# cmhungsteve/TA3N

Measured on NVIDIA H100. Metric: video-clips/sec fwd+bwd (B=256,T=5,D=2048), higher is better.
Workload: dtype tf32x3

## Files before the change

### ta3n_b200/csrc/gemm_wgmma.cuh

```cuda
#pragma once

#include <cuda.h>
#include <stdlib.h>

#include <algorithm>
#include <cmath>
#include <functional>
#include <map>
#include <tuple>

#include "seg_gemm.cuh"

namespace ta3n {

constexpr int TC_BM = 128, TC_BN = 128, TC_BK = 32;
constexpr int TC_THREADS = 288;
constexpr int TC_CONSUMER_WARPS = 8;
constexpr int TC_A_BYTES = TC_BM * TC_BK * 4;
constexpr int TC_B_BYTES = TC_BN * TC_BK * 4;
constexpr int TC_STAGE_BYTES = TC_A_BYTES + TC_B_BYTES;
constexpr int TC_STAGES = 4;
constexpr int tc_smem_bytes(int stages) { return stages * TC_STAGE_BYTES + 1024; }
constexpr int TC_ACC_LD = TC_BN + 4;
constexpr int TC_ACC_BYTES = TC_BM * TC_ACC_LD * 4;
static_assert(TC_ACC_BYTES <= TC_STAGES * TC_STAGE_BYTES, "the per-launch kernel reuses its operand ring");
#ifndef TA3N_MAX_MAPS
#define TA3N_MAX_MAPS 64
#endif
constexpr int kMaxMaps = TA3N_MAX_MAPS;

struct alignas(64) TcMaps {
  CUtensorMap m[kMaxMaps];
};
struct TcSegMaps {
  unsigned char a[kMaxSegs];
  unsigned char b[kMaxSegs];
};

__device__ __forceinline__ uint32_t smem_u32(const void* p) { return (uint32_t)__cvta_generic_to_shared(p); }

// ... 9 lines not shown
  do {
    asm volatile(
        "{\n\t.reg .pred p;\n\t"
        "mbarrier.try_wait.parity.shared::cta.b64 p, [%1], %2;\n\t"
        "selp.u32 %0, 1, 0, p;\n\t}"
        : "=r"(done)
        : "r"(addr), "r"(parity)
        : "memory");
  } while (!done);
}
__device__ __forceinline__ void mbar_arrive(uint64_t* bar) {
  asm volatile("mbarrier.arrive.shared::cta.b64 _, [%0];" ::"r"(smem_u32(bar)) : "memory");
}
__device__ __forceinline__ void fence_barrier_init() { asm volatile("fence.mbarrier_init.release.cluster;" ::: "memory"); }
__device__ __forceinline__ void fence_proxy_async() { asm volatile("fence.proxy.async.shared::cta;" ::: "memory"); }
__device__ __forceinline__ void consumer_sync() { asm volatile("bar.sync 1, 256;" ::: "memory"); }

__device__ __forceinline__ void tma_load_2d(void* smem_dst, const CUtensorMap* map, uint64_t* bar, int c0, int c1) {
  asm volatile(
      "cp.async.bulk.tensor.2d.shared::cluster.global.mbarrier::complete_tx::bytes [%0], [%1, {%3, %4}], [%2];"
      ::"r"(smem_u32(smem_dst)), "l"(map), "r"(smem_u32(bar)), "r"(c0), "r"(c1)
      : "memory");
}
__device__ __forceinline__ void tma_load_3d(void* smem_dst, const CUtensorMap* map, uint64_t* bar, int c0, int c1,
                                            int c2) {
  asm volatile(
      "cp.async.bulk.tensor.3d.shared::cluster.global.mbarrier::complete_tx::bytes [%0], [%1, {%3, %4, %5}], [%2];"
      ::"r"(smem_u32(smem_dst)), "l"(map), "r"(smem_u32(bar)), "r"(c0), "r"(c1), "r"(c2)
      : "memory");
}
__device__ __forceinline__ void tma_prefetch_2d(const CUtensorMap* map, int c0, int c1) {
// ... 71 lines not shown
  *kq = ((t >> 1) & 3) | (((t >> 7) & 1) << 2);
}
__device__ __forceinline__ void tc_prep_load(const uint32_t base, const int t, float4 (&r)[4]) {
  int mq, kq;
  tc_prep_blk(t, &mq, &kq);
#pragma unroll
  for (int i = 0; i < 4; ++i) r[i] = lds4(base + mnmaj_chunk(4 * kq + i, mq));
}
__device__ __forceinline__ void tc_prep_store(const uint32_t base, const int t, const float4 (&r)[4]) {
  int mq, kq;
  tc_prep_blk(t, &mq, &kq);
#pragma unroll
  for (int i = 0; i < 4; ++i)
    sts4(base + kmaj_chunk(4 * mq + i, kq), make_float4(f4_at(r[0], i), f4_at(r[1], i), f4_at(r[2], i), f4_at(r[3], i)));
}
__device__ __forceinline__ void tc_prep_stage(const uint32_t a_base, const uint32_t b_base, const bool a_kmaj,
                                              const bool b_kmaj) {
  if (a_kmaj && b_kmaj) return;
  const int t = threadIdx.x;
  float4 ra[4], rb[4];
  if (!a_kmaj) tc_prep_load(a_base, t, ra);
  if (!b_kmaj) tc_prep_load(b_base, t, rb);
  consumer_sync();
  if (!a_kmaj) tc_prep_store(a_base, t, ra);
  if (!b_kmaj) tc_prep_store(b_base, t, rb);
  fence_proxy_async();
  consumer_sync();
}

__device__ __forceinline__ void tc_store_acc(float* acc, const float (&d)[64], const int t) {
  const int lane = t & 31;
  const int row0 = (t >> 7) * 64 + ((t >> 5) & 3) * 16 + (lane >> 2);
#pragma unroll
  for (int j = 0; j < 16; ++j)
#pragma unroll
    for (int h = 0; h < 2; ++h)
      *reinterpret_cast<float2*>(acc + (row0 + 8 * h) * TC_ACC_LD + 8 * j + 2 * (lane & 3)) =
          make_float2(d[4 * j + 2 * h], d[4 * j + 2 * h + 1]);
}
__device__ __forceinline__ void acc_ld_32(const float* acc, int row, int col0, float* v) {
  const float* p = acc + row * TC_ACC_LD + col0;
#pragma unroll
  for (int j = 0; j < 32; j += 4) {
    const float4 q = *reinterpret_cast<const float4*>(p + j);
    v[j] = q.x;
    v[j + 1] = q.y;
    v[j + 2] = q.z;
    v[j + 3] = q.w;
  }
}

struct TcShared {
  uint64_t full_bar[4];
  uint64_t empty_bar[4];
};

template <int STAGES>
__device__ __forceinline__ void tc_pipe_init(TcShared* sh) {
  for (int s = 0; s < STAGES; ++s) {
    mbar_init(&sh->full_bar[s], 1);
    mbar_init(&sh->empty_bar[s], TC_CONSUMER_WARPS);
  }
  fence_barrier_init();
}

enum : int { TILE_FINAL = 0, TILE_PARTIAL = 1 };

template <int STAGES, int STAGE_BYTES = TC_STAGE_BYTES>
__device__ __forceinline__ void tc_produce(const TileCtx& ctx, const CUtensorMap* __restrict__ maps, const bool a_kmaj,
                                           const bool b_kmaj, const int pad_flags, const int m0, const int n0,
                                           const int c_begin, const int n_iter, uint8_t* smem, TcShared* sh,
                                           const uint32_t slabs) {
  const Group& g = ctx.g;
  int seg = 0, k0 = 0;
  {
    int skip = c_begin;
    while (seg < g.seg_count) {
      const int nch = (ctx.seg[seg].len + TC_BK - 1) / TC_BK;
      if (skip < nch) {
        k0 = skip * TC_BK;
        break;
// ... 24 lines not shown
      tma_load_2d(sB, mb, &sh->full_bar[stage], k0, n0);
    } else if (pad_flags & 2) {
      tma_load_3d(sB, mb, &sh->full_bar[stage], 0, k0, n0 >> 5);
    } else {
#pragma unroll
      for (int q = 0; q < TC_BN / 32; ++q) tma_load_2d(sB + q * 4096, mb, &sh->full_bar[stage], n0 + 32 * q, k0);
    }
    k0 += TC_BK;
    if (k0 >= ctx.seg[seg].len) {
      ++seg;
      k0 = 0;
    }
  }
}

template <int STAGES>
__device__ __forceinline__ void tc_consume(const bool a_kmaj, const bool b_kmaj, const int n_iter, uint8_t* smem,
                                           TcShared* sh, float (&d)[64]) {
  const int wg = threadIdx.x >> 7, lane = threadIdx.x & 31;
#pragma unroll
  for (int j = 0; j < 64; ++j) d[j] = 0.f;
  int prev = -1;
  for (int it = 0; it < n_iter; ++it) {
    const uint32_t gl = (uint32_t)it;
    const int stage = (int)(gl % STAGES);
    mbar_wait(&sh->full_bar[stage], (gl / STAGES) & 1u);
    const uint32_t a_base = smem_u32(smem + stage * TC_STAGE_BYTES);
    const uint32_t b_base = a_base + TC_A_BYTES;
    tc_prep_stage(a_base, b_base, a_kmaj, b_kmaj);
    wgmma_fence();
#pragma unroll
    for (int ks = 0; ks < TC_BK / 8; ++ks) wgmma_tf32(d, wgmma_desc(a_base + wg * 64 * 128, ks), wgmma_desc(b_base, ks));
    wgmma_commit();
    wgmma_wait<1>();
    if (prev >= 0) {
      __syncwarp();
      if (lane == 0) mbar_arrive(&sh->empty_bar[prev]);
    }
    prev = stage;
  }
  wgmma_wait<0>();
  if (prev >= 0) {
    __syncwarp();
    if (lane == 0) mbar_arrive(&sh->empty_bar[prev]);
  }
}

template <int kEpiWarps>
__device__ __forceinline__ void tc_epilogue(const TileCtx& ctx, const int m0, const int n0, const int split,
                                            const int n_iter, const int mode, const float* acc, const int ew) {
  const int lane = threadIdx.x & 31;
  const int lq = ew & 3;
  const Group e = ctx.g;
  const int m = m0 + lq * 32 + lane;
  const bool split_out = mode == TILE_PARTIAL;
  float* const obase = split_out ? e.partial + (size_t)split * e.M * e.N : e.C;
  const int ldo = split_out ? e.N : e.ldc;
  constexpr int kColChunks = (TC_BN / 32) * 4 / kEpiWarps;
  const int c0 = (ew / 4) * kColChunks;
#pragma unroll 1
  for (int c = c0; c < c0 + kColChunks; ++c) {
    float v[32];
    if (n_iter > 0) {
      acc_ld_32(acc, lq * 32 + lane, c * 32, v);
    } else {
#pragma unroll
      for (int j = 0; j < 32; ++j) v[j] = 0.f;
    }
    const int nb = n0 + c * 32;
    if (m < e.M && nb < e.N) {
      float* orow = obase + (size_t)m * ldo + nb;
      const int nvalid = min(32, e.N - nb);
      if (!split_out) {
        TA3N_EPI_DISPATCH(e.flags, { epilogue_row32<EPI_F>(e, m, nb, nvalid, v); })
      }
      if (nb + 32 <= e.N && ((reinterpret_cast<uintptr_t>(orow) & 15u) == 0)) {
#pragma unroll
        for (int j = 0; j < 32; j += 4)
          *reinterpret_cast<float4*>(orow + j) = make_float4(v[j], v[j + 1], v[j + 2], v[j + 3]);
      } else {
#pragma unroll
        for (int j = 0; j < 32; ++j)
          if (nb + j < e.N) orow[j] = v[j];
      }
    }
  }
}

__device__ __forceinline__ void tc_chunk_range(const TileCtx& ctx, int split, int* c_begin, int* n_iter) {
  const Group& g = ctx.g;
  int total_chunks = 0;
  for (int s = 0; s < g.seg_count; ++s) total_chunks += (ctx.seg[s].len + TC_BK - 1) / TC_BK;
  const int cps = (total_chunks + g.ksplit - 1) / g.ksplit;
  *c_begin = split * cps;
  *n_iter = max(0, min(total_chunks, *c_begin + cps) - *c_begin);
}

__device__ __forceinline__ void tc_decode(const TileCtx& ctx, const int tile, int* split, int* m0, int* n0) {
  const Group& g = ctx.g;
  int local = tile - g.tile_begin;
  const int per_split = g.tiles_m * g.tiles_n;
  *split = local / per_split;
  local -= *split * per_split;
  *m0 = (local / g.tiles_n) * TC_BM;
  *n0 = (local % g.tiles_n) * TC_BN;
}

template <bool A_KMAJ, bool B_KMAJ>
__global__ void __launch_bounds__(TC_THREADS, 1)
seg_gemm_tc_kernel(const __grid_constant__ GemmTable tab, const __grid_constant__ TcMaps maps,
                   const __grid_constant__ TcSegMaps segmaps, const int first_wave) {
  extern __shared__ uint8_t tc_smem_raw[];
  __shared__ __align__(8) TcShared sh;
  uint8_t* smem = reinterpret_cast<uint8_t*>((reinterpret_cast<uintptr_t>(tc_smem_raw) + 1023) & ~uintptr_t(1023));
  const int warp = threadIdx.x >> 5, lane = threadIdx.x & 31;

  __shared__ TileCtx ctx;
  int tile = blockIdx.x;
  if (tile >= first_wave) tile = tab.total_tiles - 1 - (tile - first_wave);
  load_tile_ctx(tab, tile, &ctx, segmaps.a, segmaps.b);
  int split, m0, n0, c_begin, n_iter;
  tc_decode(ctx, tile, &split, &m0, &n0);
  tc_chunk_range(ctx, split, &c_begin, &n_iter);

  if (warp == TC_CONSUMER_WARPS && lane == 0) tc_pipe_init<TC_STAGES>(&sh);
  __syncthreads();
  pdl_wait();

  const int mode = ctx.g.ksplit > 1 ? TILE_PARTIAL : TILE_FINAL;
  if (warp == TC_CONSUMER_WARPS) {
    if (lane == 0 && n_iter > 0)
      tc_produce<TC_STAGES>(ctx, maps.m, A_KMAJ, B_KMAJ, tab.pad_, m0, n0, c_begin, n_iter, smem, &sh, 0u);
  } else {
    float d[64];
    tc_consume<TC_STAGES>(A_KMAJ, B_KMAJ, n_iter, smem, &sh, d);
    consumer_sync();
    float* acc = reinterpret_cast<float*>(smem);
    tc_store_acc(acc, d, threadIdx.x);
    consumer_sync();
    tc_epilogue<TC_CONSUMER_WARPS>(ctx, m0, n0, split, n_iter, mode, acc, warp);
  }
}

constexpr int X3_THREADS = 384;
constexpr int X3_SPLIT_WARPS = 3;
constexpr int X3_SPLIT_THREADS = 32 * X3_SPLIT_WARPS;
constexpr int X3_PRODUCER_REGS = 40, X3_CONSUMER_REGS = 232;
static_assert(128 * X3_PRODUCER_REGS + 256 * X3_CONSUMER_REGS <= X3_THREADS * 168,
              "setmaxnreg budget exceeds the registers of one CTA");
constexpr int X3_STAGES = 4;
constexpr int X3_STAGE_BYTES = TC_STAGE_BYTES + TC_B_BYTES;
constexpr int X3_CHUNK = 8;
static_assert(X3_CHUNK % 2 == 0, "the A fragment register sets alternate by slab within a chunk");
constexpr int x3_smem_bytes() { return X3_STAGES * X3_STAGE_BYTES + 1024; }

constexpr int kX3MaxCtas = 144;
constexpr int kX3MaxTasks = 1024;
struct X3Sched {
  int listed;
  unsigned short off[kX3MaxCtas + 1];
  unsigned short task[kX3MaxTasks];
};
static_assert(sizeof(GemmTable) + sizeof(TcMaps) + sizeof(TcSegMaps) + sizeof(X3Sched) + 256 <= 32764,
              "kernel parameters of the precise kernel exceed the 32 KB limit");
// ... 34 lines not shown
  __syncwarp();
  if (lane == 0) {
    sl->ctx.gi = best;
    tc_decode(sl->ctx, tile, &sl->split, &sl->m0, &sl->n0);
    tc_chunk_range(sl->ctx, sl->split, &sl->c_begin, &sl->n_iter);
  }
  __syncwarp();
}

__device__ __forceinline__ void x3_split_sync() { asm volatile("bar.sync 2, 96;" ::: "memory"); }

template <bool B_KMAJ>
__device__ __forceinline__ void x3_split_b(const uint32_t b_raw, const uint32_t b_lo, const int t) {
  uint32_t src = b_raw;
  if (!B_KMAJ) {
#pragma unroll 1
    for (int blk = t; blk < 256; blk += X3_SPLIT_THREADS) {
      float4 r[4];
      tc_prep_load(b_raw, blk, r);
      tc_prep_store(b_lo, blk, r);
    }
    x3_split_sync();
    src = b_lo;
  }
#pragma unroll 2
  for (int c = t; c < TC_B_BYTES / 16; c += X3_SPLIT_THREADS) {
    const float4 v = lds4(src + 16u * c);
    if (!B_KMAJ) sts4(b_raw + 16u * c, v);
    sts4(b_lo + 16u * c, make_float4(v.x - tf32_hi(v.x), v.y - tf32_hi(v.y), v.z - tf32_hi(v.z), v.w - tf32_hi(v.w)));
  }
}

template <bool A_KMAJ>
__device__ __forceinline__ uint32_t x3_a_thread_off(const int m, const int tq) {
  return A_KMAJ ? kmaj_chunk(m, 0) + 4u * tq : mnmaj_chunk(tq, m >> 2) + 4u * (m & 3);
}

template <bool A_KMAJ>
__device__ __forceinline__ void x3_load_a(const uint32_t a_raw, const uint32_t off0, const uint32_t off1,
                                          uint32_t (&hi)[16], uint32_t (&lo)[16]) {
  const uint32_t p0 = a_raw + off0, p1 = a_raw + off1;
#pragma unroll
  for (int ks = 0; ks < TC_BK / 8; ++ks)
#pragma unroll
    for (int j = 0; j < 4; ++j) {
      const uint32_t row = j & 1, half = j >> 1;
      const uint32_t addr = A_KMAJ ? (p0 ^ ((2u * ks + half) << 4)) + 1024u * row
                                   : ((row ? p1 : p0) ^ (half << 6)) + 512u * half + 1024u * ks;
      const float a = lds1(addr);
      const float h = tf32_hi(a);
      hi[4 * ks + j] = __float_as_uint(h);
      lo[4 * ks + j] = __float_as_uint(a - h);
    }
#pragma unroll
  for (int j = 0; j < 16; ++j) {
    reg_fence(hi[j]);
    reg_fence(lo[j]);
  }
}

template <bool A_KMAJ>
__device__ __forceinline__ void x3_consume_slab(const uint32_t gl, uint8_t* smem, TcShared* sh, uint64_t* ready_bar,
                                                const uint32_t off0, const uint32_t off1, uint32_t (&hi)[16],
                                                uint32_t (&lo)[16], float (&d)[64], int& prev) {
// ... 9 lines not shown
  for (int ks = 0; ks < TC_BK / 8; ++ks) {
    const int f = 4 * ks;
    wgmma_tf32_rs(d, lo[f], lo[f + 1], lo[f + 2], lo[f + 3], wgmma_desc(b_hi, ks));
    wgmma_tf32_rs(d, hi[f], hi[f + 1], hi[f + 2], hi[f + 3], wgmma_desc(b_lo, ks));
    wgmma_tf32_rs(d, hi[f], hi[f + 1], hi[f + 2], hi[f + 3], wgmma_desc(b_hi, ks));
  }
  wgmma_commit();
  wgmma_wait<1>();
  if (prev >= 0) {
    __syncwarp();
    if ((threadIdx.x & 31) == 0) mbar_arrive(&sh->empty_bar[prev]);
  }
  prev = stage;
}

__device__ __forceinline__ void x3_st2(float* p, const float x0, const float x1, const bool vec, const bool two) {
  if (vec) {
    *reinterpret_cast<float2*>(p) = make_float2(x0, x1);
  } else {
    p[0] = x0;
    if (two) p[1] = x1;
  }
}

template <int F>
__device__ __forceinline__ void x3_epilogue(const Group& g, const int m0, const int n0, const float (&v)[64]) {
  constexpr bool kFwd = F >= 0 && (F & ~(EPI_BIAS | EPI_RELU | EPI_DROP_RNG)) == 0;
  const int M = g.M, N = g.N, ldc = g.ldc;
  float* const C = g.C;
  const bool vec = (N % 2) == 0 && (ldc % 2) == 0 && (reinterpret_cast<uintptr_t>(C) & 7u) == 0;
  const float alpha = kFwd ? (g.alpha_dev ? g.alpha * __ldg(g.alpha_dev) : g.alpha) : 0.f;
  const float* const bias = g.bias;
  const uint64_t seed = g.seed, roff = g.rng_offset;
  const uint64_t step = (kFwd && (F & EPI_DROP_RNG) && g.step_dev) ? *g.step_dev : 0ull;
  const float dscale = g.drop_scale, dp = g.drop_p;
  const uint32_t thr = rng_threshold(dp);
  float b0[16], b1[16];
#pragma unroll
  for (int j = 0; j < 16; ++j) {
    const int n = n0 + 8 * j;
    b0[j] = kFwd && (F & EPI_BIAS) && n < N ? bias[n] : 0.f;
    b1[j] = kFwd && (F & EPI_BIAS) && n + 1 < N ? bias[n + 1] : 0.f;
  }
#pragma unroll
  for (int h = 0; h < 2; ++h) {
    const int m = m0 + 8 * h;
    if (m >= M) continue;
#pragma unroll
    for (int j = 0; j < 16; ++j) {
      const int n = n0 + 8 * j;
      if (n >= N) continue;
      const bool two = n + 1 < N;
      float x0 = v[4 * j + 2 * h], x1 = v[4 * j + 2 * h + 1];
      if (kFwd) {
        x0 *= alpha;
        x1 *= alpha;
        if (F & EPI_BIAS) {
          x0 += b0[j];
          x1 += b1[j];
        }
        if (F & EPI_RELU) {
          x0 = fmaxf(x0, 0.0f);
          x1 = fmaxf(x1, 0.0f);
        }
        if (F & EPI_DROP_RNG) {
          const uint64_t e = roff + (uint64_t)m * (uint64_t)N + (uint64_t)n;
          bool k0, k1;
          if ((e & 1ull) == 0) {
            const uint64_t hsh = rng_hash4(seed, step, e >> 2);
            k0 = rng_keep_bits(hsh, (int)(e & 3ull), thr);
            k1 = rng_keep_bits(hsh, (int)(e & 3ull) + 1, thr);
          } else {
            k0 = rng_keep(seed, step, e, dp);
            k1 = rng_keep(seed, step, e + 1, dp);
          }
          const float f0 = k0 ? dscale : 0.0f, f1 = k1 ? dscale : 0.0f;
          x0 = f0 != 0.0f ? x0 * f0 : 0.0f;
          x1 = f1 != 0.0f ? x1 * f1 : 0.0f;
        }
      } else {
        x0 = epilogue_t<F>(g, m, n, x0);
        if (two) x1 = epilogue_t<F>(g, m, n + 1, x1);
      }
      x3_st2(C + (size_t)m * ldc + n, x0, x1, vec, two);
    }
  }
}

__device__ __forceinline__ void x3_finish(const X3Slot& sl, const float (&v)[64]) {
  const Group& g = sl.ctx.g;
  const int warp = threadIdx.x >> 5, lane = threadIdx.x & 31;
  const int m0 = sl.m0 + (warp >> 2) * 64 + (warp & 3) * 16 + (lane >> 2), n0 = sl.n0 + 2 * (lane & 3);
  if (g.ksplit > 1) {
    const int M = g.M, N = g.N;
    float* const part = g.partial + (size_t)sl.split * M * N;
    const bool vec = (N % 2) == 0;
#pragma unroll
    for (int h = 0; h < 2; ++h)
#pragma unroll
      for (int j = 0; j < 16; ++j) {
        const int m = m0 + 8 * h, n = n0 + 8 * j;
        if (m < M && n < N) x3_st2(part + (size_t)m * N + n, v[4 * j + 2 * h], v[4 * j + 2 * h + 1], vec, n + 1 < N);
      }
    return;
  }
  TA3N_EPI_DISPATCH(g.flags, { x3_epilogue<EPI_F>(g, m0, n0, v); })
}

template <bool A_KMAJ, bool B_KMAJ>
__global__ void __launch_bounds__(X3_THREADS, 1)
seg_gemm_tc_x3_kernel(const __grid_constant__ GemmTable tab, const __grid_constant__ TcMaps maps,
                      const __grid_constant__ TcSegMaps segmaps, const __grid_constant__ X3Sched sched) {
  extern __shared__ uint8_t tc_smem_raw[];
  __shared__ __align__(8) TcShared sh;
  __shared__ __align__(8) uint64_t ready_bar[X3_STAGES];
  __shared__ __align__(8) uint64_t slot_full[2], slot_empty[2];
  __shared__ X3Slot slots[2];
  uint8_t* smem = reinterpret_cast<uint8_t*>((reinterpret_cast<uintptr_t>(tc_smem_raw) + 1023) & ~uintptr_t(1023));
  const int warp = threadIdx.x >> 5, lane = threadIdx.x & 31;
  const int n_tasks = sched.listed ? sched.off[blockIdx.x + 1] - sched.off[blockIdx.x]
                                   : (tab.total_tiles - (int)blockIdx.x + (int)gridDim.x - 1) / (int)gridDim.x;

  if (warp == TC_CONSUMER_WARPS) {
    if (lane == 0) {
      for (int s = 0; s < X3_STAGES; ++s) mbar_init(&ready_bar[s], X3_SPLIT_WARPS);
      for (int s = 0; s < 2; ++s) {
        mbar_init(&slot_full[s], 1);
        mbar_init(&slot_empty[s], X3_SLOT_READERS);
      }
      tc_pipe_init<X3_STAGES>(&sh);
    }
    __syncwarp();
    x3_stage(tab, segmaps, x3_task(sched, 0), &slots[0]);
    if (lane == 0) mbar_arrive(&slot_full[0]);
  }
  __syncthreads();
  pdl_wait();

  if (warp >= TC_CONSUMER_WARPS) {
    setmaxnreg_dec<X3_PRODUCER_REGS>();
    uint32_t slabs = 0;
    if (warp == TC_CONSUMER_WARPS) {
      for (int k = 0; k < n_tasks; ++k) {
        const int s = k & 1;
        if (k > 0) {
          mbar_wait(&slot_empty[s], ((uint32_t)(k >> 1) & 1u) ^ 1u);
          x3_stage(tab, segmaps, x3_task(sched, k), &slots[s]);
          if (lane == 0) mbar_arrive(&slot_full[s]);
        }
        const X3Slot& sl = slots[s];
        if (lane == 0 && sl.n_iter > 0)
          tc_produce<X3_STAGES, X3_STAGE_BYTES>(sl.ctx, maps.m, A_KMAJ, B_KMAJ, tab.pad_, sl.m0, sl.n0, sl.c_begin,
                                                sl.n_iter, smem, &sh, slabs);
        __syncwarp();
        slabs += (uint32_t)sl.n_iter;
// ... 8 lines not shown
        if (lane == 0) mbar_arrive(&slot_empty[s]);
        for (int it = 0; it < n_iter; ++it) {
          const uint32_t gl = slabs + (uint32_t)it;
          const int stage = (int)(gl % X3_STAGES);
          mbar_wait(&sh.full_bar[stage], (gl / X3_STAGES) & 1u);
          const uint32_t b_raw = smem_u32(smem + stage * X3_STAGE_BYTES) + TC_A_BYTES;
          x3_split_b<B_KMAJ>(b_raw, b_raw + TC_B_BYTES, t);
          fence_proxy_async();
          __syncwarp();
          if (lane == 0) mbar_arrive(&ready_bar[stage]);
        }
        slabs += (uint32_t)n_iter;
      }
    }
  } else {
    setmaxnreg_inc<X3_CONSUMER_REGS>();
    const int r0 = (warp >> 2) * 64 + (warp & 3) * 16 + (lane >> 2);
    const uint32_t off0 = x3_a_thread_off<A_KMAJ>(r0, lane & 3), off1 = x3_a_thread_off<A_KMAJ>(r0 + 8, lane & 3);
    uint32_t slabs = 0;
    for (int k = 0; k < n_tasks; ++k) {
      const int s = k & 1;
      mbar_wait(&slot_full[s], (uint32_t)(k >> 1) & 1u);
      const int n_iter = slots[s].n_iter;
      float d[64], sum[64];
#pragma unroll
      for (int j = 0; j < 64; ++j) d[j] = sum[j] = 0.f;
      uint32_t hi[2][16], lo[2][16];
      int prev = -1;
      for (int c0 = 0; c0 < n_iter; c0 += X3_CHUNK) {
        const int c1 = min(n_iter, c0 + X3_CHUNK);
        for (int it = c0; it < c1; it += 2) {
          x3_consume_slab<A_KMAJ>(slabs + (uint32_t)it, smem, &sh, ready_bar, off0, off1, hi[0], lo[0], d, prev);
          if (it + 1 < c1)
            x3_consume_slab<A_KMAJ>(slabs + (uint32_t)(it + 1), smem, &sh, ready_bar, off0, off1, hi[1], lo[1], d, prev);
        }
        wgmma_wait<0>();
        __syncwarp();
        if (lane == 0) mbar_arrive(&sh.empty_bar[prev]);
        prev = -1;
#pragma unroll
        for (int j = 0; j < 64; ++j) {
          sum[j] += d[j];
          d[j] = 0.f;
        }
      }
      slabs += (uint32_t)n_iter;
      x3_finish(slots[s], sum);
      __syncwarp();
      if (lane == 0) mbar_arrive(&slot_empty[s]);
    }
  }
}

typedef CUresult (*PFN_encodeTiled)(CUtensorMap*, CUtensorMapDataType, cuuint32_t, void*, const cuuint64_t*,
                                    const cuuint64_t*, const cuuint32_t*, const cuuint32_t*, CUtensorMapInterleave,
                                    CUtensorMapSwizzle, CUtensorMapL2promotion, CUtensorMapFloatOOBfill);

inline PFN_encodeTiled encode_fn() {
  static PFN_encodeTiled fn = []() -> PFN_encodeTiled {
    void* p = nullptr;
    cudaDriverEntryPointQueryResult q;
    if (cudaGetDriverEntryPoint("cuTensorMapEncodeTiled", &p, cudaEnableDefault, &q) != cudaSuccess) return nullptr;
    if (q != cudaDriverEntryPointSuccess) return nullptr;
    return reinterpret_cast<PFN_encodeTiled>(p);
  }();
// ... 89 lines not shown
  *ka = a_kmaj ? MapKey{s.A, s.len, g.M, s.lda, TC_BK, TC_BM, 0, rw} : MapKey{s.A, g.M, s.len, s.lda, 32, TC_BK, a3d ? 1 : 0, rw};
  *kb = b_kmaj ? MapKey{s.B, s.len, g.N, s.ldb, TC_BK, TC_BN, 0, rw} : MapKey{s.B, g.N, s.len, s.ldb, 32, TC_BK, b3d ? 1 : 0, rw};
}

template <bool A_KMAJ, bool B_KMAJ>
inline int tc_launch_one(const GemmTable& tab, const TcMaps& maps, const TcSegMaps& sm, cudaStream_t stream,
                         const char* label) {
  constexpr int slot = (A_KMAJ ? 0 : 1) + (B_KMAJ ? 0 : 2);
  int first_wave = 132;
  {
    std::lock_guard<std::mutex> lock(device_mu());
    DeviceInfo* d = device_info();
    if (!d) return fail(TA3N_ERR_CUDA, "cudaGetDevice failed");
    if (!d->configured[slot]) {
      TA3N_CUDA(cudaFuncSetAttribute(seg_gemm_tc_kernel<A_KMAJ, B_KMAJ>, cudaFuncAttributeMaxDynamicSharedMemorySize,
                                     tc_smem_bytes(TC_STAGES)));
      d->configured[slot] = true;
    }
    first_wave = d->sm_count;
  }
  pre_launch(label, stream);
  launch_kernel(seg_gemm_tc_kernel<A_KMAJ, B_KMAJ>, tab.total_tiles, TC_THREADS, tc_smem_bytes(TC_STAGES), stream, tab,
                maps, sm, first_wave);
  return after_launch();
}

template <bool A_KMAJ, bool B_KMAJ>
inline int tc_launch_x3(const GemmTable& tab, const TcMaps& maps, const TcSegMaps& sm, const X3Sched& sched, int grid,
                        cudaStream_t stream, const char* label) {
  constexpr int slot = (A_KMAJ ? 0 : 1) + (B_KMAJ ? 0 : 2);
  {
    std::lock_guard<std::mutex> lock(device_mu());
    DeviceInfo* d = device_info();
    if (!d) return fail(TA3N_ERR_CUDA, "cudaGetDevice failed");
    if (!d->x3_configured[slot]) {
      TA3N_CUDA(cudaFuncSetAttribute(seg_gemm_tc_x3_kernel<A_KMAJ, B_KMAJ>, cudaFuncAttributeMaxDynamicSharedMemorySize,
                                     x3_smem_bytes()));
      d->x3_configured[slot] = true;
    }
  }
  pre_launch(label, stream);
  launch_kernel(seg_gemm_tc_x3_kernel<A_KMAJ, B_KMAJ>, grid, X3_THREADS, x3_smem_bytes(), stream, tab, maps, sm, sched);
  return after_launch();
}

inline GemmPlan sub_plan(const GemmPlan& plan, const std::vector<int>& idx) {
  GemmPlan out;
  out.a_kmaj = plan.a_kmaj;
  out.b_kmaj = plan.b_kmaj;
  out.load_flags = plan.load_flags;
  out.label = plan.label;
  for (int i : idx) {
    Group g = plan.groups[i];
    const int b = g.seg_begin;
    g.seg_begin = (int)out.segs.size();
    for (int k = 0; k < g.seg_count; ++k) out.segs.push_back(plan.segs[b + k]);
    out.groups.push_back(g);
// ... 282 lines not shown
```

Measured before the change: 1.071 million.

## Restructure per-launch TF32 GEMM kernel with warp-specialized B transpose and register-fed A

```diff
diff --git a/ta3n_b200/csrc/gemm_wgmma.cuh b/ta3n_b200/csrc/gemm_wgmma.cuh
--- a/ta3n_b200/csrc/gemm_wgmma.cuh
+++ b/ta3n_b200/csrc/gemm_wgmma.cuh
@@ -14,16 +14,19 @@
 namespace ta3n {
 
 constexpr int TC_BM = 128, TC_BN = 128, TC_BK = 32;
-constexpr int TC_THREADS = 288;
+constexpr int TC_THREADS = 384;
 constexpr int TC_CONSUMER_WARPS = 8;
+constexpr int TC_B_WARPS = 3;
+constexpr int TC_B_THREADS = 32 * TC_B_WARPS;
+constexpr int TC_PRODUCER_REGS = 40, TC_CONSUMER_REGS = 232;
+static_assert(128 * TC_PRODUCER_REGS + 256 * TC_CONSUMER_REGS <= TC_THREADS * 168,
+              "setmaxnreg budget exceeds the registers of one CTA");
 constexpr int TC_A_BYTES = TC_BM * TC_BK * 4;
 constexpr int TC_B_BYTES = TC_BN * TC_BK * 4;
 constexpr int TC_STAGE_BYTES = TC_A_BYTES + TC_B_BYTES;
 constexpr int TC_STAGES = 4;
-constexpr int tc_smem_bytes(int stages) { return stages * TC_STAGE_BYTES + 1024; }
-constexpr int TC_ACC_LD = TC_BN + 4;
-constexpr int TC_ACC_BYTES = TC_BM * TC_ACC_LD * 4;
-static_assert(TC_ACC_BYTES <= TC_STAGES * TC_STAGE_BYTES, "the per-launch kernel reuses its operand ring");
+__host__ __device__ constexpr int tc_stage_bytes(bool b_kmaj) { return TC_STAGE_BYTES + (b_kmaj ? 0 : TC_B_BYTES); }
+constexpr int tc_smem_bytes(bool b_kmaj) { return TC_STAGES * tc_stage_bytes(b_kmaj) + 1024; }
 #ifndef TA3N_MAX_MAPS
 #define TA3N_MAX_MAPS 64
 #endif
@@ -63,7 +66,6 @@
 }
 __device__ __forceinline__ void fence_barrier_init() { asm volatile("fence.mbarrier_init.release.cluster;" ::: "memory"); }
 __device__ __forceinline__ void fence_proxy_async() { asm volatile("fence.proxy.async.shared::cta;" ::: "memory"); }
-__device__ __forceinline__ void consumer_sync() { asm volatile("bar.sync 1, 256;" ::: "memory"); }
 
 __device__ __forceinline__ void tma_load_2d(void* smem_dst, const CUtensorMap* map, uint64_t* bar, int c0, int c1) {
   asm volatile(
@@ -165,39 +167,12 @@
   for (int i = 0; i < 4; ++i)
     sts4(base + kmaj_chunk(4 * mq + i, kq), make_float4(f4_at(r[0], i), f4_at(r[1], i), f4_at(r[2], i), f4_at(r[3], i)));
 }
-__device__ __forceinline__ void tc_prep_stage(const uint32_t a_base, const uint32_t b_base, const bool a_kmaj,
-                                              const bool b_kmaj) {
-  if (a_kmaj && b_kmaj) return;
-  const int t = threadIdx.x;
-  float4 ra[4], rb[4];
-  if (!a_kmaj) tc_prep_load(a_base, t, ra);
-  if (!b_kmaj) tc_prep_load(b_base, t, rb);
-  consumer_sync();
-  if (!a_kmaj) tc_prep_store(a_base, t, ra);
-  if (!b_kmaj) tc_prep_store(b_base, t, rb);
-  fence_proxy_async();
-  consumer_sync();
-}
-
-__device__ __forceinline__ void tc_store_acc(float* acc, const float (&d)[64], const int t) {
-  const int lane = t & 31;
-  const int row0 = (t >> 7) * 64 + ((t >> 5) & 3) * 16 + (lane >> 2);
-#pragma unroll
-  for (int j = 0; j < 16; ++j)
-#pragma unroll
-    for (int h = 0; h < 2; ++h)
-      *reinterpret_cast<float2*>(acc + (row0 + 8 * h) * TC_ACC_LD + 8 * j + 2 * (lane & 3)) =
-          make_float2(d[4 * j + 2 * h], d[4 * j + 2 * h + 1]);
-}
-__device__ __forceinline__ void acc_ld_32(const float* acc, int row, int col0, float* v) {
-  const float* p = acc + row * TC_ACC_LD + col0;
-#pragma unroll
-  for (int j = 0; j < 32; j += 4) {
-    const float4 q = *reinterpret_cast<const float4*>(p + j);
-    v[j] = q.x;
-    v[j + 1] = q.y;
-    v[j + 2] = q.z;
-    v[j + 3] = q.w;
+__device__ __forceinline__ void tc_transpose_b(const uint32_t b_raw, const uint32_t b_kmaj, const int t) {
+#pragma unroll 1
+  for (int blk = t; blk < 256; blk += TC_B_THREADS) {
+    float4 r[4];
+    tc_prep_load(b_raw, blk, r);
+    tc_prep_store(b_kmaj, blk, r);
   }
 }
 
@@ -214,8 +189,6 @@
   }
   fence_barrier_init();
 }
-
-enum : int { TILE_FINAL = 0, TILE_PARTIAL = 1 };
 
 template <int STAGES, int STAGE_BYTES = TC_STAGE_BYTES>
 __device__ __forceinline__ void tc_produce(const TileCtx& ctx, const CUtensorMap* __restrict__ maps, const bool a_kmaj,
@@ -270,79 +243,6 @@
   }
 }
 
-template <int STAGES>
-__device__ __forceinline__ void tc_consume(const bool a_kmaj, const bool b_kmaj, const int n_iter, uint8_t* smem,
-                                           TcShared* sh, float (&d)[64]) {
-  const int wg = threadIdx.x >> 7, lane = threadIdx.x & 31;
-#pragma unroll
-  for (int j = 0; j < 64; ++j) d[j] = 0.f;
-  int prev = -1;
-  for (int it = 0; it < n_iter; ++it) {
-    const uint32_t gl = (uint32_t)it;
-    const int stage = (int)(gl % STAGES);
-    mbar_wait(&sh->full_bar[stage], (gl / STAGES) & 1u);
-    const uint32_t a_base = smem_u32(smem + stage * TC_STAGE_BYTES);
-    const uint32_t b_base = a_base + TC_A_BYTES;
-    tc_prep_stage(a_base, b_base, a_kmaj, b_kmaj);
-    wgmma_fence();
-#pragma unroll
-    for (int ks = 0; ks < TC_BK / 8; ++ks) wgmma_tf32(d, wgmma_desc(a_base + wg * 64 * 128, ks), wgmma_desc(b_base, ks));
-    wgmma_commit();
-    wgmma_wait<1>();
-    if (prev >= 0) {
-      __syncwarp();
-      if (lane == 0) mbar_arrive(&sh->empty_bar[prev]);
-    }
-    prev = stage;
-  }
-  wgmma_wait<0>();
-  if (prev >= 0) {
-    __syncwarp();
-    if (lane == 0) mbar_arrive(&sh->empty_bar[prev]);
-  }
-}
-
-template <int kEpiWarps>
-__device__ __forceinline__ void tc_epilogue(const TileCtx& ctx, const int m0, const int n0, const int split,
-                                            const int n_iter, const int mode, const float* acc, const int ew) {
-  const int lane = threadIdx.x & 31;
-  const int lq = ew & 3;
-  const Group e = ctx.g;
-  const int m = m0 + lq * 32 + lane;
-  const bool split_out = mode == TILE_PARTIAL;
-  float* const obase = split_out ? e.partial + (size_t)split * e.M * e.N : e.C;
-  const int ldo = split_out ? e.N : e.ldc;
-  constexpr int kColChunks = (TC_BN / 32) * 4 / kEpiWarps;
-  const int c0 = (ew / 4) * kColChunks;
-#pragma unroll 1
-  for (int c = c0; c < c0 + kColChunks; ++c) {
-    float v[32];
-    if (n_iter > 0) {
-      acc_ld_32(acc, lq * 32 + lane, c * 32, v);
-    } else {
-#pragma unroll
-      for (int j = 0; j < 32; ++j) v[j] = 0.f;
-    }
-    const int nb = n0 + c * 32;
-    if (m < e.M && nb < e.N) {
-      float* orow = obase + (size_t)m * ldo + nb;
-      const int nvalid = min(32, e.N - nb);
-      if (!split_out) {
-        TA3N_EPI_DISPATCH(e.flags, { epilogue_row32<EPI_F>(e, m, nb, nvalid, v); })
-      }
-      if (nb + 32 <= e.N && ((reinterpret_cast<uintptr_t>(orow) & 15u) == 0)) {
-#pragma unroll
-        for (int j = 0; j < 32; j += 4)
-          *reinterpret_cast<float4*>(orow + j) = make_float4(v[j], v[j + 1], v[j + 2], v[j + 3]);
-      } else {
-#pragma unroll
-        for (int j = 0; j < 32; ++j)
-          if (nb + j < e.N) orow[j] = v[j];
-      }
-    }
-  }
-}
-
 __device__ __forceinline__ void tc_chunk_range(const TileCtx& ctx, int split, int* c_begin, int* n_iter) {
   const Group& g = ctx.g;
   int total_chunks = 0;
@@ -362,48 +262,6 @@
   *n0 = (local % g.tiles_n) * TC_BN;
 }
 
-template <bool A_KMAJ, bool B_KMAJ>
-__global__ void __launch_bounds__(TC_THREADS, 1)
-seg_gemm_tc_kernel(const __grid_constant__ GemmTable tab, const __grid_constant__ TcMaps maps,
-                   const __grid_constant__ TcSegMaps segmaps, const int first_wave) {
-  extern __shared__ uint8_t tc_smem_raw[];
-  __shared__ __align__(8) TcShared sh;
-  uint8_t* smem = reinterpret_cast<uint8_t*>((reinterpret_cast<uintptr_t>(tc_smem_raw) + 1023) & ~uintptr_t(1023));
-  const int warp = threadIdx.x >> 5, lane = threadIdx.x & 31;
-
-  __shared__ TileCtx ctx;
-  int tile = blockIdx.x;
-  if (tile >= first_wave) tile = tab.total_tiles - 1 - (tile - first_wave);
-  load_tile_ctx(tab, tile, &ctx, segmaps.a, segmaps.b);
-  int split, m0, n0, c_begin, n_iter;
-  tc_decode(ctx, tile, &split, &m0, &n0);
-  tc_chunk_range(ctx, split, &c_begin, &n_iter);
-
-  if (warp == TC_CONSUMER_WARPS && lane == 0) tc_pipe_init<TC_STAGES>(&sh);
-  __syncthreads();
-  pdl_wait();
-
-  const int mode = ctx.g.ksplit > 1 ? TILE_PARTIAL : TILE_FINAL;
-  if (warp == TC_CONSUMER_WARPS) {
-    if (lane == 0 && n_iter > 0)
-      tc_produce<TC_STAGES>(ctx, maps.m, A_KMAJ, B_KMAJ, tab.pad_, m0, n0, c_begin, n_iter, smem, &sh, 0u);
-  } else {
-    float d[64];
-    tc_consume<TC_STAGES>(A_KMAJ, B_KMAJ, n_iter, smem, &sh, d);
-    consumer_sync();
-    float* acc = reinterpret_cast<float*>(smem);
-    tc_store_acc(acc, d, threadIdx.x);
-    consumer_sync();
-    tc_epilogue<TC_CONSUMER_WARPS>(ctx, m0, n0, split, n_iter, mode, acc, warp);
-  }
-}
-
-constexpr int X3_THREADS = 384;
-constexpr int X3_SPLIT_WARPS = 3;
-constexpr int X3_SPLIT_THREADS = 32 * X3_SPLIT_WARPS;
-constexpr int X3_PRODUCER_REGS = 40, X3_CONSUMER_REGS = 232;
-static_assert(128 * X3_PRODUCER_REGS + 256 * X3_CONSUMER_REGS <= X3_THREADS * 168,
-              "setmaxnreg budget exceeds the registers of one CTA");
 constexpr int X3_STAGES = 4;
 constexpr int X3_STAGE_BYTES = TC_STAGE_BYTES + TC_B_BYTES;
 constexpr int X3_CHUNK = 8;
@@ -468,17 +326,12 @@
 __device__ __forceinline__ void x3_split_b(const uint32_t b_raw, const uint32_t b_lo, const int t) {
   uint32_t src = b_raw;
   if (!B_KMAJ) {
-#pragma unroll 1
-    for (int blk = t; blk < 256; blk += X3_SPLIT_THREADS) {
-      float4 r[4];
-      tc_prep_load(b_raw, blk, r);
-      tc_prep_store(b_lo, blk, r);
-    }
+    tc_transpose_b(b_raw, b_lo, t);
     x3_split_sync();
     src = b_lo;
   }
 #pragma unroll 2
-  for (int c = t; c < TC_B_BYTES / 16; c += X3_SPLIT_THREADS) {
+  for (int c = t; c < TC_B_BYTES / 16; c += TC_B_THREADS) {
     const float4 v = lds4(src + 16u * c);
     if (!B_KMAJ) sts4(b_raw + 16u * c, v);
     sts4(b_lo + 16u * c, make_float4(v.x - tf32_hi(v.x), v.y - tf32_hi(v.y), v.z - tf32_hi(v.z), v.w - tf32_hi(v.w)));
@@ -486,8 +339,15 @@
 }
 
 template <bool A_KMAJ>
-__device__ __forceinline__ uint32_t x3_a_thread_off(const int m, const int tq) {
+__device__ __forceinline__ uint32_t tc_a_thread_off(const int m, const int tq) {
   return A_KMAJ ? kmaj_chunk(m, 0) + 4u * tq : mnmaj_chunk(tq, m >> 2) + 4u * (m & 3);
+}
+
+template <bool A_KMAJ>
+__device__ __forceinline__ uint32_t tc_a_addr(const uint32_t p0, const uint32_t p1, const int ks, const int j) {
+  const uint32_t row = j & 1, half = j >> 1;
+  return A_KMAJ ? (p0 ^ ((2u * ks + half) << 4)) + 1024u * row
+                : ((row ? p1 : p0) ^ (half << 6)) + 512u * half + 1024u * ks;
 }
 
 template <bool A_KMAJ>
@@ -498,10 +358,7 @@
   for (int ks = 0; ks < TC_BK / 8; ++ks)
 #pragma unroll
     for (int j = 0; j < 4; ++j) {
-      const uint32_t row = j & 1, half = j >> 1;
-      const uint32_t addr = A_KMAJ ? (p0 ^ ((2u * ks + half) << 4)) + 1024u * row
-                                   : ((row ? p1 : p0) ^ (half << 6)) + 512u * half + 1024u * ks;
-      const float a = lds1(addr);
+      const float a = lds1(tc_a_addr<A_KMAJ>(p0, p1, ks, j));
       const float h = tf32_hi(a);
       hi[4 * ks + j] = __float_as_uint(h);
       lo[4 * ks + j] = __float_as_uint(a - h);
@@ -541,7 +398,7 @@
   prev = stage;
 }
 
-__device__ __forceinline__ void x3_st2(float* p, const float x0, const float x1, const bool vec, const bool two) {
+__device__ __forceinline__ void tc_st2(float* p, const float x0, const float x1, const bool vec, const bool two) {
   if (vec) {
     *reinterpret_cast<float2*>(p) = make_float2(x0, x1);
   } else {
@@ -550,24 +407,141 @@
   }
 }
 
+__device__ __forceinline__ void tc_drop_row(const Group& g, const int f, const int m, const int n0, float (&x)[32]) {
+  const int N = g.N;
+  if (f & EPI_DROP_MASK) {
+    const uint8_t* k = g.keep + (size_t)m * g.ldkeep;
+#pragma unroll
+    for (int i = 0; i < 32; ++i) {
+      const int n = n0 + 8 * (i >> 1) + (i & 1);
+      if (n < N) x[i] = k[n] ? x[i] * g.drop_scale : 0.0f;
+    }
+  }
+  if (f & EPI_DROP_RNG) {
+    const uint64_t step = g.step_dev ? *g.step_dev : 0ull;
+    const uint32_t thr = rng_threshold(g.drop_p);
+#pragma unroll
+    for (int j = 0; j < 16; ++j) {
+      const uint64_t e = g.rng_offset + (uint64_t)m * (uint64_t)N + (uint64_t)(n0 + 8 * j);
+      bool k0, k1;
+      if ((e & 1ull) == 0) {
+        const uint64_t hsh = rng_hash4(g.seed, step, e >> 2);
+        k0 = rng_keep_bits(hsh, (int)(e & 3ull), thr);
+        k1 = rng_keep_bits(hsh, (int)(e & 3ull) + 1, thr);
+      } else {
+        k0 = rng_keep(g.seed, step, e, g.drop_p);
+        k1 = rng_keep(g.seed, step, e + 1, g.drop_p);
+      }
+      x[2 * j] = k0 ? x[2 * j] * g.drop_scale : 0.0f;
+      x[2 * j + 1] = k1 ? x[2 * j + 1] * g.drop_scale : 0.0f;
+    }
+  }
+}
+
 template <int F>
-__device__ __forceinline__ void x3_epilogue(const Group& g, const int m0, const int n0, const float (&v)[64]) {
+__device__ __forceinline__ void tc_epilogue_bwd(const Group& gs, const int m0, const int n0, const float (&v)[64]) {
+  const Group g = gs;
+  const int f = F >= 0 ? F : g.flags;
+  const int M = g.M, N = g.N;
+  const bool vec = (N % 2) == 0 && (g.ldc % 2) == 0 && (reinterpret_cast<uintptr_t>(g.C) & 7u) == 0;
+  const float alpha = g.alpha_dev ? g.alpha * __ldg(g.alpha_dev) : g.alpha;
+#pragma unroll
+  for (int h = 0; h < 2; ++h) {
+    const int m = m0 + 8 * h;
+    if (m >= M) continue;
+    float x[32], a_bias[32], a_add[32], a_gate[32], a_c[32];
+    float rs = 1.0f;
+    if ((f & EPI_ADDROW) && g.rowscale) rs = __ldcg(g.rowscale + (size_t)m * g.rs_stride) + g.rs_bias;
+#pragma unroll
+    for (int i = 0; i < 32; ++i) {
+      const int n = n0 + 8 * (i >> 1) + (i & 1);
+      const bool ok = n < N;
+      if (f & EPI_BIAS) a_bias[i] = ok ? __ldcg(g.bias + n) : 0.f;
+      if (f & EPI_ADDROW) a_add[i] = ok ? __ldcg(g.add + (size_t)m * g.ldadd + n) : 0.f;
+      if (f & (EPI_GATE | EPI_DPRE)) a_gate[i] = ok ? __ldcg(g.gate + (size_t)m * g.ldgate + n) : 0.f;
+      if (f & EPI_ACCUM) a_c[i] = ok ? __ldcg(g.C + (size_t)m * g.ldc + n) : 0.f;
+      x[i] = v[4 * (i >> 1) + 2 * h + (i & 1)];
+    }
+#pragma unroll
+    for (int i = 0; i < 32; ++i) x[i] *= alpha;
+    if (f & EPI_BIAS) {
+#pragma unroll
+      for (int i = 0; i < 32; ++i) x[i] += a_bias[i];
+    }
+    if (f & EPI_RELU) {
+#pragma unroll
+      for (int i = 0; i < 32; ++i) x[i] = fmaxf(x[i], 0.0f);
+    }
+    if ((f & (EPI_DROP_MASK | EPI_DROP_RNG)) && !(f & EPI_DROP_LATE)) tc_drop_row(g, f, m, n0, x);
+    if (f & EPI_ADDROW) {
+#pragma unroll
+      for (int i = 0; i < 32; ++i) x[i] = fmaf(rs, a_add[i], x[i]);
+    }
+    if ((f & (EPI_DROP_MASK | EPI_DROP_RNG)) && (f & EPI_DROP_LATE)) tc_drop_row(g, f, m, n0, x);
+    if (f & EPI_GATE) {
+#pragma unroll
+      for (int i = 0; i < 32; ++i) x[i] = a_gate[i] > 0.0f ? x[i] : 0.0f;
+    }
+    if (f & EPI_ACCUM) {
+#pragma unroll
+      for (int i = 0; i < 32; ++i) x[i] += a_c[i];
+    }
+    if (f & EPI_DPRE) {
+#pragma unroll
+      for (int i = 0; i < 32; ++i) x[i] = a_gate[i] > 0.0f ? x[i] * g.drop_scale : 0.0f;
+    }
+    if (f & EPI_MULTI) {
+      const bool vm = (g.ldmulti % 2) == 0;
+#pragma unroll
+      for (int q = 0; q < 3; ++q) {
+        if (q >= g.n_multi) break;
+        const float* gq = g.multi_gate[q] + (size_t)m * g.ldmulti;
+        float* oq = g.multi_out[q] + (size_t)m * g.ldmulti;
+        float a_mg[32];
+#pragma unroll
+        for (int i = 0; i < 32; ++i) {
+          const int n = n0 + 8 * (i >> 1) + (i & 1);
+          a_mg[i] = n < N ? __ldcg(gq + n) : 0.f;
+        }
+        const bool vq = vm && (reinterpret_cast<uintptr_t>(oq) & 7u) == 0;
+#pragma unroll
+        for (int j = 0; j < 16; ++j) {
+          const int n = n0 + 8 * j;
+          if (n < N)
+            tc_st2(oq + n, a_mg[2 * j] > 0.f ? x[2 * j] : 0.f, a_mg[2 * j + 1] > 0.f ? x[2 * j + 1] : 0.f, vq, n + 1 < N);
+        }
+      }
+    }
+#pragma unroll
+    for (int j = 0; j < 16; ++j) {
+      const int n = n0 + 8 * j;
+      if (n < N) tc_st2(g.C + (size_t)m * g.ldc + n, x[2 * j], x[2 * j + 1], vec, n + 1 < N);
+    }
+  }
+}
+
+template <int F>
+__device__ __forceinline__ void tc_epilogue(const Group& g, const int m0, const int n0, const float (&v)[64]) {
   constexpr bool kFwd = F >= 0 && (F & ~(EPI_BIAS | EPI_RELU | EPI_DROP_RNG)) == 0;
+  if (!kFwd) {
+    tc_epilogue_bwd<F>(g, m0, n0, v);
+    return;
+  }
   const int M = g.M, N = g.N, ldc = g.ldc;
   float* const C = g.C;
   const bool vec = (N % 2) == 0 && (ldc % 2) == 0 && (reinterpret_cast<uintptr_t>(C) & 7u) == 0;
-  const float alpha = kFwd ? (g.alpha_dev ? g.alpha * __ldg(g.alpha_dev) : g.alpha) : 0.f;
+  const float alpha = g.alpha_dev ? g.alpha * __ldg(g.alpha_dev) : g.alpha;
   const float* const bias = g.bias;
   const uint64_t seed = g.seed, roff = g.rng_offset;
-  const uint64_t step = (kFwd && (F & EPI_DROP_RNG) && g.step_dev) ? *g.step_dev : 0ull;
+  const uint64_t step = ((F & EPI_DROP_RNG) && g.step_dev) ? *g.step_dev : 0ull;
   const float dscale = g.drop_scale, dp = g.drop_p;
   const uint32_t thr = rng_threshold(dp);
   float b0[16], b1[16];
 #pragma unroll
   for (int j = 0; j < 16; ++j) {
     const int n = n0 + 8 * j;
-    b0[j] = kFwd && (F & EPI_BIAS) && n < N ? bias[n] : 0.f;
-    b1[j] = kFwd && (F & EPI_BIAS) && n + 1 < N ? bias[n + 1] : 0.f;
+    b0[j] = (F & EPI_BIAS) && n < N ? bias[n] : 0.f;
+    b1[j] = (F & EPI_BIAS) && n + 1 < N ? bias[n + 1] : 0.f;
   }
 #pragma unroll
   for (int h = 0; h < 2; ++h) {
@@ -579,63 +553,58 @@
       if (n >= N) continue;
       const bool two = n + 1 < N;
       float x0 = v[4 * j + 2 * h], x1 = v[4 * j + 2 * h + 1];
-      if (kFwd) {
-        x0 *= alpha;
-        x1 *= alpha;
-        if (F & EPI_BIAS) {
-          x0 += b0[j];
-          x1 += b1[j];
+      x0 *= alpha;
+      x1 *= alpha;
+      if (F & EPI_BIAS) {
+        x0 += b0[j];
+        x1 += b1[j];
+      }
+      if (F & EPI_RELU) {
+        x0 = fmaxf(x0, 0.0f);
+        x1 = fmaxf(x1, 0.0f);
+      }
+      if (F & EPI_DROP_RNG) {
+        const uint64_t e = roff + (uint64_t)m * (uint64_t)N + (uint64_t)n;
+        bool k0, k1;
+        if ((e & 1ull) == 0) {
+          const uint64_t hsh = rng_hash4(seed, step, e >> 2);
+          k0 = rng_keep_bits(hsh, (int)(e & 3ull), thr);
+          k1 = rng_keep_bits(hsh, (int)(e & 3ull) + 1, thr);
+        } else {
+          k0 = rng_keep(seed, step, e, dp);
+          k1 = rng_keep(seed, step, e + 1, dp);
         }
-        if (F & EPI_RELU) {
-          x0 = fmaxf(x0, 0.0f);
-          x1 = fmaxf(x1, 0.0f);
-        }
-        if (F & EPI_DROP_RNG) {
-          const uint64_t e = roff + (uint64_t)m * (uint64_t)N + (uint64_t)n;
-          bool k0, k1;
-          if ((e & 1ull) == 0) {
-            const uint64_t hsh = rng_hash4(seed, step, e >> 2);
-            k0 = rng_keep_bits(hsh, (int)(e & 3ull), thr);
-            k1 = rng_keep_bits(hsh, (int)(e & 3ull) + 1, thr);
-          } else {
-            k0 = rng_keep(seed, step, e, dp);
-            k1 = rng_keep(seed, step, e + 1, dp);
-          }
-          const float f0 = k0 ? dscale : 0.0f, f1 = k1 ? dscale : 0.0f;
-          x0 = f0 != 0.0f ? x0 * f0 : 0.0f;
-          x1 = f1 != 0.0f ? x1 * f1 : 0.0f;
-        }
-      } else {
-        x0 = epilogue_t<F>(g, m, n, x0);
-        if (two) x1 = epilogue_t<F>(g, m, n + 1, x1);
-      }
-      x3_st2(C + (size_t)m * ldc + n, x0, x1, vec, two);
-    }
-  }
-}
-
-__device__ __forceinline__ void x3_finish(const X3Slot& sl, const float (&v)[64]) {
-  const Group& g = sl.ctx.g;
+        const float f0 = k0 ? dscale : 0.0f, f1 = k1 ? dscale : 0.0f;
+        x0 = f0 != 0.0f ? x0 * f0 : 0.0f;
+        x1 = f1 != 0.0f ? x1 * f1 : 0.0f;
+      }
+      tc_st2(C + (size_t)m * ldc + n, x0, x1, vec, two);
+    }
+  }
+}
+
+__device__ __forceinline__ void tc_finish(const Group& g, const int split, const int tm0, const int tn0,
+                                          const float (&v)[64]) {
   const int warp = threadIdx.x >> 5, lane = threadIdx.x & 31;
-  const int m0 = sl.m0 + (warp >> 2) * 64 + (warp & 3) * 16 + (lane >> 2), n0 = sl.n0 + 2 * (lane & 3);
+  const int m0 = tm0 + (warp >> 2) * 64 + (warp & 3) * 16 + (lane >> 2), n0 = tn0 + 2 * (lane & 3);
   if (g.ksplit > 1) {
     const int M = g.M, N = g.N;
-    float* const part = g.partial + (size_t)sl.split * M * N;
+    float* const part = g.partial + (size_t)split * M * N;
     const bool vec = (N % 2) == 0;
 #pragma unroll
     for (int h = 0; h < 2; ++h)
 #pragma unroll
       for (int j = 0; j < 16; ++j) {
         const int m = m0 + 8 * h, n = n0 + 8 * j;
-        if (m < M && n < N) x3_st2(part + (size_t)m * N + n, v[4 * j + 2 * h], v[4 * j + 2 * h + 1], vec, n + 1 < N);
+        if (m < M && n < N) tc_st2(part + (size_t)m * N + n, v[4 * j + 2 * h], v[4 * j + 2 * h + 1], vec, n + 1 < N);
       }
     return;
   }
-  TA3N_EPI_DISPATCH(g.flags, { x3_epilogue<EPI_F>(g, m0, n0, v); })
+  TA3N_EPI_DISPATCH(g.flags, { tc_epilogue<EPI_F>(g, m0, n0, v); })
 }
 
 template <bool A_KMAJ, bool B_KMAJ>
-__global__ void __launch_bounds__(X3_THREADS, 1)
+__global__ void __launch_bounds__(TC_THREADS, 1)
 seg_gemm_tc_x3_kernel(const __grid_constant__ GemmTable tab, const __grid_constant__ TcMaps maps,
                       const __grid_constant__ TcSegMaps segmaps, const __grid_constant__ X3Sched sched) {
   extern __shared__ uint8_t tc_smem_raw[];
@@ -650,7 +619,7 @@
 
   if (warp == TC_CONSUMER_WARPS) {
     if (lane == 0) {
-      for (int s = 0; s < X3_STAGES; ++s) mbar_init(&ready_bar[s], X3_SPLIT_WARPS);
+      for (int s = 0; s < X3_STAGES; ++s) mbar_init(&ready_bar[s], TC_B_WARPS);
       for (int s = 0; s < 2; ++s) {
         mbar_init(&slot_full[s], 1);
         mbar_init(&slot_empty[s], X3_SLOT_READERS);
@@ -665,7 +634,7 @@
   pdl_wait();
 
   if (warp >= TC_CONSUMER_WARPS) {
-    setmaxnreg_dec<X3_PRODUCER_REGS>();
+    setmaxnreg_dec<TC_PRODUCER_REGS>();
     uint32_t slabs = 0;
     if (warp == TC_CONSUMER_WARPS) {
       for (int k = 0; k < n_tasks; ++k) {
@@ -704,9 +673,9 @@
       }
     }
   } else {
-    setmaxnreg_inc<X3_CONSUMER_REGS>();
+    setmaxnreg_inc<TC_CONSUMER_REGS>();
     const int r0 = (warp >> 2) * 64 + (warp & 3) * 16 + (lane >> 2);
-    const uint32_t off0 = x3_a_thread_off<A_KMAJ>(r0, lane & 3), off1 = x3_a_thread_off<A_KMAJ>(r0 + 8, lane & 3);
+    const uint32_t off0 = tc_a_thread_off<A_KMAJ>(r0, lane & 3), off1 = tc_a_thread_off<A_KMAJ>(r0 + 8, lane & 3);
     uint32_t slabs = 0;
     for (int k = 0; k < n_tasks; ++k) {
       const int s = k & 1;
@@ -735,10 +704,111 @@
         }
       }
       slabs += (uint32_t)n_iter;
-      x3_finish(slots[s], sum);
+      tc_finish(slots[s].ctx.g, slots[s].split, slots[s].m0, slots[s].n0, sum);
       __syncwarp();
       if (lane == 0) mbar_arrive(&slot_empty[s]);
     }
+  }
+}
+
+__device__ __forceinline__ void tc_load_a(const uint32_t a_base, const uint32_t off0, const uint32_t off1,
+                                          uint32_t (&a)[16]) {
+  const uint32_t p0 = a_base + off0, p1 = a_base + off1;
+#pragma unroll
+  for (int ks = 0; ks < TC_BK / 8; ++ks)
+#pragma unroll
+    for (int j = 0; j < 4; ++j) a[4 * ks + j] = __float_as_uint(lds1(tc_a_addr<false>(p0, p1, ks, j)));
+#pragma unroll
+  for (int j = 0; j < 16; ++j) reg_fence(a[j]);
+}
+
+template <bool A_KMAJ, bool B_KMAJ>
+__device__ __forceinline__ void tc_consume_slab(const int it, uint8_t* smem, TcShared* sh, uint64_t* ready_bar,
+                                                const uint32_t off0, const uint32_t off1, uint32_t (&a)[16],
+                                                float (&d)[64], int& prev) {
+  const int stage = it % TC_STAGES;
+  const uint32_t parity = (uint32_t)(it / TC_STAGES) & 1u;
+  mbar_wait(&sh->full_bar[stage], parity);
+  if (!B_KMAJ) mbar_wait(&ready_bar[stage], parity);
+  const uint32_t a_base = smem_u32(smem + stage * tc_stage_bytes(B_KMAJ));
+  const uint32_t b_base = a_base + TC_A_BYTES + (B_KMAJ ? 0 : TC_B_BYTES);
+  if (!A_KMAJ) tc_load_a(a_base, off0, off1, a);
+  wgmma_fence();
+#pragma unroll
+  for (int ks = 0; ks < TC_BK / 8; ++ks) {
+    if (A_KMAJ)
+      wgmma_tf32(d, wgmma_desc(a_base + (threadIdx.x >> 7) * 64 * 128, ks), wgmma_desc(b_base, ks));
+    else
+      wgmma_tf32_rs(d, a[4 * ks], a[4 * ks + 1], a[4 * ks + 2], a[4 * ks + 3], wgmma_desc(b_base, ks));
+  }
+  wgmma_commit();
+  wgmma_wait<1>();
+  if (prev >= 0) {
+    __syncwarp();
+    if ((threadIdx.x & 31) == 0) mbar_arrive(&sh->empty_bar[prev]);
+  }
+  prev = stage;
+}
+
+template <bool A_KMAJ, bool B_KMAJ>
+__global__ void __launch_bounds__(TC_THREADS, 1)
+seg_gemm_tc_kernel(const __grid_constant__ GemmTable tab, const __grid_constant__ TcMaps maps,
+                   const __grid_constant__ TcSegMaps segmaps, const int first_wave) {
+  extern __shared__ uint8_t tc_smem_raw[];
+  __shared__ __align__(8) TcShared sh;
+  __shared__ __align__(8) uint64_t ready_bar[TC_STAGES];
+  uint8_t* smem = reinterpret_cast<uint8_t*>((reinterpret_cast<uintptr_t>(tc_smem_raw) + 1023) & ~uintptr_t(1023));
+  const int warp = threadIdx.x >> 5, lane = threadIdx.x & 31;
+
+  __shared__ TileCtx ctx;
+  int tile = blockIdx.x;
+  if (tile >= first_wave) tile = tab.total_tiles - 1 - (tile - first_wave);
+  load_tile_ctx(tab, tile, &ctx, segmaps.a, segmaps.b);
+  int split, m0, n0, c_begin, n_iter;
+  tc_decode(ctx, tile, &split, &m0, &n0);
+  tc_chunk_range(ctx, split, &c_begin, &n_iter);
+
+  if (warp == TC_CONSUMER_WARPS && lane == 0) {
+    if (!B_KMAJ)
+      for (int s = 0; s < TC_STAGES; ++s) mbar_init(&ready_bar[s], TC_B_WARPS);
+    tc_pipe_init<TC_STAGES>(&sh);
+  }
+  __syncthreads();
+  pdl_wait();
+
+  if (warp >= TC_CONSUMER_WARPS) {
+    setmaxnreg_dec<TC_PRODUCER_REGS>();
+    if (warp == TC_CONSUMER_WARPS) {
+      if (lane == 0 && n_iter > 0)
+        tc_produce<TC_STAGES, tc_stage_bytes(B_KMAJ)>(ctx, maps.m, A_KMAJ, B_KMAJ, tab.pad_, m0, n0, c_begin, n_iter,
+                                                      smem, &sh, 0u);
+    } else if (!B_KMAJ) {
+      const int t = threadIdx.x - 32 * (TC_CONSUMER_WARPS + 1);
+      for (int it = 0; it < n_iter; ++it) {
+        const int stage = it % TC_STAGES;
+        mbar_wait(&sh.full_bar[stage], (uint32_t)(it / TC_STAGES) & 1u);
+        const uint32_t b_raw = smem_u32(smem + stage * tc_stage_bytes(B_KMAJ)) + TC_A_BYTES;
+        tc_transpose_b(b_raw, b_raw + TC_B_BYTES, t);
+        fence_proxy_async();
+        __syncwarp();
+        if (lane == 0) mbar_arrive(&ready_bar[stage]);
+      }
+    }
+  } else {
+    setmaxnreg_inc<TC_CONSUMER_REGS>();
+    const int r0 = (warp >> 2) * 64 + (warp & 3) * 16 + (lane >> 2);
+    const uint32_t off0 = tc_a_thread_off<false>(r0, lane & 3), off1 = tc_a_thread_off<false>(r0 + 8, lane & 3);
+    float d[64];
+#pragma unroll
+    for (int j = 0; j < 64; ++j) d[j] = 0.f;
+    uint32_t a[2][16];
+    int prev = -1;
+    for (int it = 0; it < n_iter; it += 2) {
+      tc_consume_slab<A_KMAJ, B_KMAJ>(it, smem, &sh, ready_bar, off0, off1, a[0], d, prev);
+      if (it + 1 < n_iter) tc_consume_slab<A_KMAJ, B_KMAJ>(it + 1, smem, &sh, ready_bar, off0, off1, a[1], d, prev);
+    }
+    wgmma_wait<0>();
+    tc_finish(ctx.g, split, m0, n0, d);
   }
 }
 
@@ -858,13 +928,13 @@
     if (!d) return fail(TA3N_ERR_CUDA, "cudaGetDevice failed");
     if (!d->configured[slot]) {
       TA3N_CUDA(cudaFuncSetAttribute(seg_gemm_tc_kernel<A_KMAJ, B_KMAJ>, cudaFuncAttributeMaxDynamicSharedMemorySize,
-                                     tc_smem_bytes(TC_STAGES)));
+                                     tc_smem_bytes(B_KMAJ)));
       d->configured[slot] = true;
     }
     first_wave = d->sm_count;
   }
   pre_launch(label, stream);
-  launch_kernel(seg_gemm_tc_kernel<A_KMAJ, B_KMAJ>, tab.total_tiles, TC_THREADS, tc_smem_bytes(TC_STAGES), stream, tab,
+  launch_kernel(seg_gemm_tc_kernel<A_KMAJ, B_KMAJ>, tab.total_tiles, TC_THREADS, tc_smem_bytes(B_KMAJ), stream, tab,
                 maps, sm, first_wave);
   return after_launch();
 }
@@ -884,7 +954,7 @@
     }
   }
   pre_launch(label, stream);
-  launch_kernel(seg_gemm_tc_x3_kernel<A_KMAJ, B_KMAJ>, grid, X3_THREADS, x3_smem_bytes(), stream, tab, maps, sm, sched);
+  launch_kernel(seg_gemm_tc_x3_kernel<A_KMAJ, B_KMAJ>, grid, TC_THREADS, x3_smem_bytes(), stream, tab, maps, sm, sched);
   return after_launch();
 }
 
```

After: 1.154 million, median of 6. +7.8%, better.
